# bioscan-ml/bioscan-clip

Hardware: AMD Instinct MI355X
Metric: paired samples/sec/node (I+D+T, global batch) + step MFMA-roofline % at 1/2/4/8 GPU (higher is better)
Workload: dtype bf16; 1 GPU; configs[2]: Image+DNA+Text (LoRA ViT-B/16 + LoRA BarcodeBERT + BERT-small), local batch 256, 224x224 images + 133-token barcodes, local-batch InfoNCE, fused AdamW; local_batch=256, global_batch=256, parallelism=dp1, collectives=none (one process, local-batch loss)

## Files before the change

### bioscan-clip_amd/csrc/optim.hip

```cpp
#include <math.h>

#include <type_traits>

#include "common.h"

namespace {

typedef __attribute__((ext_vector_type(4))) unsigned u32x4;

__device__ __forceinline__ f32x4 ld_bf4(const bf16_t* p) {
    const uint2 u = *reinterpret_cast<const uint2*>(p);
    return f32x4{bf2f(u.x & 0xffff), bf2f(u.x >> 16), bf2f(u.y & 0xffff), bf2f(u.y >> 16)};
}

__device__ __forceinline__ float reduce8(float (&p)[8], int lane) {
    float q[4];
    const bool hi5 = lane & 32;
#pragma unroll
    for (int i = 0; i < 4; ++i) {
        const float send = hi5 ? p[i] : p[i + 4];
        const float keep = hi5 ? p[i + 4] : p[i];
        q[i] = keep + __shfl_xor(send, 32, 64);
    }
    float r2[2];
    const bool hi4 = lane & 16;
#pragma unroll
    for (int i = 0; i < 2; ++i) {
        const float send = hi4 ? q[i] : q[i + 2];
        const float keep = hi4 ? q[i + 2] : q[i];
        r2[i] = keep + __shfl_xor(send, 16, 64);
    }
    const bool hi3 = lane & 8;
    float v = (hi3 ? r2[1] : r2[0]) + __shfl_xor(hi3 ? r2[0] : r2[1], 8, 64);
    v += __shfl_xor(v, 4, 64);
    v += __shfl_xor(v, 2, 64);
    v += __shfl_xor(v, 1, 64);
    return v;
}

constexpr int LG_BLOCK = 256;

__device__ __forceinline__ f32x4 splat4(float v) {
    f32x4 s = {v, v, v, v};
    asm("" : "+v"(s));
    return s;
}

__device__ __forceinline__ float reduce4(float (&p)[4], int lane) {
    float q[2];
    const bool hi5 = lane & 32;
#pragma unroll
    for (int i = 0; i < 2; ++i) {
        const float send = hi5 ? p[i] : p[i + 2];
        const float keep = hi5 ? p[i + 2] : p[i];
        q[i] = keep + __shfl_xor(send, 32, 64);
    }
    const bool hi4 = lane & 16;
    float v = (hi4 ? q[1] : q[0]) + __shfl_xor(hi4 ? q[0] : q[1], 16, 64);
    v += __shfl_xor(v, 8, 64);
    v += __shfl_xor(v, 4, 64);
    v += __shfl_xor(v, 2, 64);
    v += __shfl_xor(v, 1, 64);
    return v;
}

template <int H, bool F32IN = false>
__global__ __launch_bounds__(LG_BLOCK) void lora_grad_dt_db_kernel(const void* __restrict__ dqkv_, int ld,
                                                                    const void* __restrict__ haug_, int ld_h, int M,
                                                                    const float* __restrict__ lora_b,
                                                                    float* __restrict__ dt,
                                                                    float* __restrict__ partial) {
    const bf16_t* dqkv = static_cast<const bf16_t*>(dqkv_);
    const bf16_t* haug = static_cast<const bf16_t*>(haug_);
    constexpr int NV = H / 256;
    __shared__ float red[2 * NV * 16 * 64];
    const int lane = threadIdx.x & 63;
    const int wib = __builtin_amdgcn_readfirstlane(threadIdx.x >> 6);
    const int is_v = wib & 1;
    const int pair = blockIdx.x * (LG_BLOCK / 128) + (wib >> 1);
    const int npairs = gridDim.x * (LG_BLOCK / 128);
    for (int i = threadIdx.x; i < 2 * NV * 16 * 64; i += LG_BLOCK) red[i] = 0.f;

    f32x4 bx[NV][4];
    f32x4 ax[NV][4];
#pragma unroll
    for (int j = 0; j < NV; ++j)
#pragma unroll
        for (int i = 0; i < 4; ++i) {
            const int c = j * 256 + lane * 4 + i;
            bx[j][i] = *reinterpret_cast<const f32x4*>(lora_b + (size_t)(is_v * H + c) * 4);
            ax[j][i] = f32x4{0.f, 0.f, 0.f, 0.f};
        }

    constexpr int PF = 3;
    using row_t = std::conditional_t<F32IN, f32x4, uint2>;
    row_t rx[PF][NV];
    row_t rt[PF];
    auto fetch = [&](int slot, int row) {
        if constexpr (F32IN) {
            const float* g = static_cast<const float*>(dqkv_) + (size_t)row * ld + is_v * 2 * H;
#pragma unroll
            for (int j = 0; j < NV; ++j) rx[slot][j] = *reinterpret_cast<const f32x4*>(g + j * 256 + lane * 4);
            rt[slot] = *reinterpret_cast<const f32x4*>(static_cast<const float*>(haug_) + (size_t)row * ld_h + 4 * is_v);
        } else {
            const bf16_t* g = dqkv + (size_t)row * ld + is_v * 2 * H;
#pragma unroll
            for (int j = 0; j < NV; ++j) rx[slot][j] = *reinterpret_cast<const uint2*>(g + j * 256 + lane * 4);
            rt[slot] = *reinterpret_cast<const uint2*>(haug + (size_t)row * ld_h + H + 4 * is_v);
        }
    };
#pragma unroll
    for (int p = 0; p < PF; ++p)
        if (pair + p * npairs < M) fetch(p, pair + p * npairs);
    auto body = [&](int slot, int row) {
        f32x4 dx[NV];
        f32x4 tx;
        if constexpr (F32IN) {
#pragma unroll
            for (int j = 0; j < NV; ++j) dx[j] = rx[slot][j];
            tx = rt[slot];
        } else {
#pragma unroll
            for (int j = 0; j < NV; ++j)
                dx[j] = f32x4{bf2f(rx[slot][j].x & 0xffff), bf2f(rx[slot][j].x >> 16), bf2f(rx[slot][j].y & 0xffff),
                              bf2f(rx[slot][j].y >> 16)};
            const uint2 tu = rt[slot];
            tx = f32x4{bf2f(tu.x & 0xffff), bf2f(tu.x >> 16), bf2f(tu.y & 0xffff), bf2f(tu.y >> 16)};
        }
        if (row + PF * npairs < M) fetch(slot, row + PF * npairs);
        f32x4 px = {0.f, 0.f, 0.f, 0.f};
#pragma unroll
        for (int j = 0; j < NV; ++j)
#pragma unroll
            for (int i = 0; i < 4; ++i) {
                const f32x4 d4 = splat4(dx[j][i]);
                px += d4 * bx[j][i];
                ax[j][i] += d4 * tx;
            }
        float p[4] = {px[0], px[1], px[2], px[3]};
        const float tot = reduce4(p, lane);
        const float tl = __shfl(tot, ((lane >> 1) & 1) * 32 + (lane & 1) * 16, 64);
        if (lane < 4) dt[(size_t)row * 8 + 4 * is_v + lane] = tl;
    };
    for (int row = pair; row < M; row += PF * npairs) {
#pragma unroll
        for (int p = 0; p < PF; ++p)
            if (row + p * npairs < M) body(p, row + p * npairs);
    }
    float* mine = red + is_v * (NV * 16 * 64);
    for (int w = 0; w < LG_BLOCK / 64; ++w) {
        __syncthreads();
        if (wib == w) {
#pragma unroll
            for (int j = 0; j < NV; ++j)
#pragma unroll
                for (int i = 0; i < 4; ++i)
#pragma unroll
                    for (int r = 0; r < 4; ++r) mine[((j * 16 + i * 4 + r) * 64) + lane] += ax[j][i][r];
        }
    }
    __syncthreads();
    for (int idx = threadIdx.x; idx < 2 * NV * 16 * 64; idx += LG_BLOCK)
        partial[(size_t)blockIdx.x * (2 * NV * 16 * 64) + idx] = red[idx];
}

template <int H, bool Y_FP8 = false, bool Y_F32 = false, bool F16 = false>
__global__ __launch_bounds__(LG_BLOCK) void lora_grad_da_kernel(const void* __restrict__ haug_, int ld_h, int M,
                                                                 const float* __restrict__ dt,
                                                                 float* __restrict__ partial) {
    const bf16_t* haug = static_cast<const bf16_t*>(haug_);
    constexpr int NV = H / 256;
    __shared__ float red[8 * NV * 4 * 64];
    const int lane = threadIdx.x & 63;
    const int wave = (blockIdx.x * LG_BLOCK + threadIdx.x) >> 6;
    const int nwaves = (gridDim.x * LG_BLOCK) >> 6;
    for (int i = threadIdx.x; i < 8 * NV * 4 * 64; i += LG_BLOCK) red[i] = 0.f;
    f32x4 acc[8][NV];
#pragma unroll
    for (int r = 0; r < 8; ++r)
#pragma unroll
        for (int j = 0; j < NV; ++j) acc[r][j] = f32x4{0.f, 0.f, 0.f, 0.f};
    constexpr int PF = 3;
    for (int row0 = wave; row0 < M; row0 += PF * nwaves) {
        f32x4 d0[PF], d1[PF];
        std::conditional_t<Y_F32, f32x4, uint2> yr[PF][NV];
#pragma unroll
        for (int p = 0; p < PF; ++p) {
            const int row = min(row0 + p * nwaves, M - 1);
            d0[p] = *reinterpret_cast<const f32x4*>(dt + (size_t)row * 8);
            d1[p] = *reinterpret_cast<const f32x4*>(dt + (size_t)row * 8 + 4);
#pragma unroll
            for (int j = 0; j < NV; ++j) {
                if constexpr (Y_F32) {
                    yr[p][j] = *reinterpret_cast<const f32x4*>(static_cast<const float*>(haug_) + (size_t)row * ld_h + j * 256 + lane * 4);
                } else if constexpr (Y_FP8) {
                    yr[p][j].x = *reinterpret_cast<const unsigned*>(reinterpret_cast<const unsigned char*>(haug) +
                                                                    (size_t)row * ld_h + j * 256 + lane * 4);
                    yr[p][j].y = 0;
                } else {
                    yr[p][j] = *reinterpret_cast<const uint2*>(haug + (size_t)row * ld_h + j * 256 + lane * 4);
                }
            }
        }
#pragma unroll
        for (int p = 0; p < PF; ++p) {
            if (row0 + p * nwaves >= M) break;
#pragma unroll
            for (int j = 0; j < NV; ++j) {
                f32x4 y;
                if constexpr (Y_F32)
                    y = yr[p][j];
                else if constexpr (Y_FP8)
                    y = f32x4{fp8_to_f32(yr[p][j].x, 0), fp8_to_f32(yr[p][j].x, 1), fp8_to_f32(yr[p][j].x, 2), fp8_to_f32(yr[p][j].x, 3)};
                else
                    y = f32x4{h2f<F16>(yr[p][j].x & 0xffff), h2f<F16>(yr[p][j].x >> 16), h2f<F16>(yr[p][j].y & 0xffff),
                              h2f<F16>(yr[p][j].y >> 16)};
#pragma unroll
                for (int r = 0; r < 4; ++r) {
                    acc[r][j] += splat4(d0[p][r]) * y;
                    acc[4 + r][j] += splat4(d1[p][r]) * y;
                }
            }
        }
    }
    const int wib = threadIdx.x >> 6;
    for (int w = 0; w < LG_BLOCK / 64; ++w) {
        __syncthreads();
        if (wib == w) {
#pragma unroll
            for (int r = 0; r < 8; ++r)
#pragma unroll
                for (int j = 0; j < NV; ++j)
#pragma unroll
                    for (int i = 0; i < 4; ++i) red[(((r * NV + j) * 4 + i) * 64) + lane] += acc[r][j][i];
        }
    }
    __syncthreads();
    for (int idx = threadIdx.x; idx < 8 * NV * 4 * 64; idx += LG_BLOCK)
        partial[(size_t)blockIdx.x * (8 * NV * 4 * 64) + idx] = red[idx];
}

template <int H>
__global__ __launch_bounds__(LG_BLOCK) void lora_t_f32_kernel(const float* __restrict__ y, int ld_y, int M, const float* __restrict__ A,
                                                              float* __restrict__ t) {
    constexpr int NV = H / 256;
    __shared__ __attribute__((aligned(16))) float sA[8 * H];
    for (int i = threadIdx.x * 4; i < 8 * H; i += LG_BLOCK * 4) *reinterpret_cast<f32x4*>(sA + i) = *reinterpret_cast<const f32x4*>(A + i);
    __syncthreads();
    const int lane = threadIdx.x & 63;
    const int wave = (blockIdx.x * LG_BLOCK + threadIdx.x) >> 6, nwaves = (gridDim.x * LG_BLOCK) >> 6;
    for (int row = wave; row < M; row += nwaves) {
        asm volatile("" ::: "memory");
        f32x4 v[NV];
#pragma unroll
        for (int j = 0; j < NV; ++j) v[j] = *reinterpret_cast<const f32x4*>(y + (size_t)row * ld_y + j * 256 + lane * 4);
        float p[8];
#pragma unroll
        for (int r = 0; r < 8; ++r) {
            float d = 0.f;
#pragma unroll
            for (int j = 0; j < NV; ++j) {
                const f32x4 a = *reinterpret_cast<const f32x4*>(sA + r * H + j * 256 + lane * 4);
                d += (v[j][0] * a[0] + v[j][1] * a[1]) + (v[j][2] * a[2] + v[j][3] * a[3]);
            }
            p[r] = d;
        }
        const float tt = reduce8(p, lane);
        const float tl = __shfl(tt, ((lane >> 2) & 1) * 32 + ((lane >> 1) & 1) * 16 + (lane & 1) * 8, 64);
        if (lane < 8) t[(size_t)row * 8 + lane] = tl;
    }
}

template <int H, bool UNSCALE = false>
__global__ __launch_bounds__(256) void lora_grad_reduce_kernel(const float* __restrict__ pa,
                                                                const float* __restrict__ pb, int nblocks,
                                                                float* __restrict__ dA, float* __restrict__ dBq,
                                                                float* __restrict__ dBv, int first_block = 0, float unscale = 1.f) {
    constexpr int NV = H / 256;
    constexpr int SLAB = 8 * H;
    __shared__ f32x4 red[32][8];
    const int q = threadIdx.x & 7, p = threadIdx.x >> 3;
    const int idx = (blockIdx.x + first_block) * 32 + q * 4;
    const bool second = idx >= SLAB;
    const int e = second ? idx - SLAB : idx;
    const float* src = (second ? pb : pa) + e;
    f32x4 s = {0.f, 0.f, 0.f, 0.f};
    int b = p;
    for (; b + 96 < nblocks; b += 128) {
        f32x4 v[4];
#pragma unroll
        for (int u = 0; u < 4; ++u) v[u] = *reinterpret_cast<const f32x4*>(src + (size_t)(b + 32 * u) * SLAB);
#pragma unroll
        for (int u = 0; u < 4; ++u) s += v[u];
    }
    for (; b < nblocks; b += 32) s += *reinterpret_cast<const f32x4*>(src + (size_t)b * SLAB);
    red[p][q] = s;
    __syncthreads();
    if (p != 0) return;
    s = red[0][q];
#pragma unroll
    for (int g = 1; g < 32; ++g) s += red[g][q];
    if constexpr (UNSCALE) s *= unscale;
#pragma unroll
    for (int c = 0; c < 4; ++c) {
        const int ec = e + c;
        const int l = ec & 63, k = ec >> 6;
        if (!second) {
            const bool is_v = k >= NV * 16;
            const int kk = is_v ? k - NV * 16 : k;
            const int j = kk >> 4, ii = (kk >> 2) & 3, r = kk & 3;
            const int col = j * 256 + l * 4 + ii;
            float* dst = (is_v ? dBv : dBq) + (size_t)col * 4 + r;
            *dst += s[c];
        } else {
            const int ii = k & 3, j = (k >> 2) % NV, r = (k >> 2) / NV;
            dA[(size_t)r * H + j * 256 + l * 4 + ii] += s[c];
        }
    }
}

template <bool UNSCALE = false>
__global__ __launch_bounds__(256) void lora_heads_reduce_kernel(const float* __restrict__ dtp, const float* __restrict__ dbp, int M,
                                                                 int heads, int items, int nA, float* __restrict__ dt,
                                                                 float* __restrict__ dBq, float* __restrict__ dBv, float unscale = 1.f) {
    if ((int)blockIdx.x < nA) {
        const int g = blockIdx.x * 256 + threadIdx.x, row = g >> 1, half = g & 1;
        if (row >= M) return;
        f32x4 s = {0.f, 0.f, 0.f, 0.f};
        for (int hd = 0; hd < heads; hd += 4) {
            f32x4 v[4];
#pragma unroll
            for (int u = 0; u < 4; ++u) v[u] = *reinterpret_cast<const f32x4*>(dtp + (((size_t)(hd + u) * 2 + half) * M + row) * 4);
#pragma unroll
            for (int u = 0; u < 4; ++u) s += v[u];
        }
        *reinterpret_cast<f32x4*>(dt + (size_t)row * 8 + 4 * half) = s;
        return;
    }
    __shared__ float red[8][32];
    const int i = threadIdx.x & 31, p = threadIdx.x >> 5;
    const int e = ((int)blockIdx.x - nA) * 32 + i;
    const size_t stride = (size_t)heads * 512;
    const float* src = dbp + e;
    float s = 0.f;
    int b = p;
    for (; b + 56 < items; b += 64) {
        float v[8];
#pragma unroll
        for (int u = 0; u < 8; ++u) v[u] = src[(size_t)(b + 8 * u) * stride];
#pragma unroll
        for (int u = 0; u < 8; ++u) s += v[u];
    }
    for (; b < items; b += 8) s += src[(size_t)b * stride];
    red[p][i] = s;
    __syncthreads();
    if (p != 0) return;
    s = ((red[0][i] + red[1][i]) + (red[2][i] + red[3][i])) + ((red[4][i] + red[5][i]) + (red[6][i] + red[7][i]));
    if constexpr (UNSCALE) s *= unscale;
    const int hd = e >> 9, is_v = (e >> 8) & 1, j = (e >> 6) & 3, d = e & 63;
    float* dst = (is_v ? dBv : dBq) + (size_t)(hd * 64 + d) * 4 + j;
    *dst += s;
}

template <bool BF16>
__global__ __launch_bounds__(256) void colsum8_kernel(const void* __restrict__ g, int ld, int M, int N,
                                                       float* __restrict__ out) {
    __shared__ float part[256][9];
    __shared__ float part2[8][8];
    const int t = threadIdx.x;
    const int n0 = blockIdx.x * 8;
    float s[8] = {0.f, 0.f, 0.f, 0.f, 0.f, 0.f, 0.f, 0.f};
    auto add_row = [&](int r) {
        if constexpr (BF16) {
            const u32x4 u = *reinterpret_cast<const u32x4*>(static_cast<const bf16_t*>(g) + (size_t)r * ld + n0);
#pragma unroll
            for (int k = 0; k < 4; ++k) {
                s[2 * k] += bf2f(u[k] & 0xffff);
                s[2 * k + 1] += bf2f(u[k] >> 16);
            }
        } else {
            const float* p = static_cast<const float*>(g) + (size_t)r * ld + n0;
            const f32x4 a = *reinterpret_cast<const f32x4*>(p), b = *reinterpret_cast<const f32x4*>(p + 4);
#pragma unroll
            for (int k = 0; k < 4; ++k) {
                s[k] += a[k];
                s[4 + k] += b[k];
            }
        }
    };
    int r = t;
    for (; r + 768 < M; r += 1024) {
        add_row(r);
        add_row(r + 256);
        add_row(r + 512);
        add_row(r + 768);
    }
    for (; r < M; r += 256) add_row(r);
#pragma unroll
    for (int k = 0; k < 8; ++k) part[t][k] = s[k];
    __syncthreads();
    if (t < 64) {
        const int c = t & 7, o = t >> 3;
        float a = 0.f;
        for (int i = 0; i < 32; ++i) a += part[32 * o + i][c];
        part2[o][c] = a;
    }
    __syncthreads();
    if (t < 8) {
        float a = 0.f;
#pragma unroll
        for (int o = 0; o < 8; ++o) a += part2[o][t];
        out[n0 + t] += a;
    }
}

template <bool BF16>
__global__ __launch_bounds__(256) void colsum_kernel(const void* __restrict__ g, int ld, int M, int N,
                                                      float* __restrict__ out) {
    __shared__ float part[8][32];
    const int c = threadIdx.x & 31, rg = threadIdx.x >> 5;
    const int n = blockIdx.x * 32 + c;
    float s[4] = {0.f, 0.f, 0.f, 0.f};
    if (n < N) {
        auto at = [&](int r) -> float {
            if constexpr (BF16) return bf2f(static_cast<const bf16_t*>(g)[(size_t)r * ld + n]);
            else return static_cast<const float*>(g)[(size_t)r * ld + n];
        };
        int r = rg;
        for (; r + 24 < M; r += 32) {
#pragma unroll
            for (int u = 0; u < 4; ++u) s[u] += at(r + 8 * u);
        }
        for (; r < M; r += 8) s[0] += at(r);
    }
    part[rg][c] = (s[0] + s[1]) + (s[2] + s[3]);
    __syncthreads();
    if (rg == 0 && n < N) {
        float t = 0.f;
#pragma unroll
        for (int k = 0; k < 8; ++k) t += part[k][c];
        out[n] += t;
    }
}

__global__ __launch_bounds__(256) void adamw_kernel(float* __restrict__ p, const float* __restrict__ g,
                                                     float* __restrict__ m, float* __restrict__ v, long n, float lr,
                                                     float beta1, float beta2, float eps, float wd, float inv_bc1,
                                                     float inv_sqrt_bc2, float grad_scale) {
    for (long i = (long)blockIdx.x * 256 + threadIdx.x; i < n; i += (long)gridDim.x * 256) {
        const float gi = g[i] * grad_scale;
        float pi = p[i] * (1.0f - lr * wd);
        const float mi = beta1 * m[i] + (1.0f - beta1) * gi;
        const float vi = beta2 * v[i] + (1.0f - beta2) * gi * gi;
        const float denom = sqrtf(vi) * inv_sqrt_bc2 + eps;
        pi -= (lr * inv_bc1) * (mi / denom);
        p[i] = pi;
        m[i] = mi;
        v[i] = vi;
    }
}

__global__ __launch_bounds__(256) void adamw_dev_kernel(float* __restrict__ p, const float* __restrict__ g,
                                                         float* __restrict__ m, float* __restrict__ v, long n,
                                                         const float* __restrict__ hyper, float beta1, float beta2, float eps,
                                                         float wd, float grad_scale) {
    const float lr = hyper[0];
    const double step = (double)reinterpret_cast<const unsigned*>(hyper)[1];
    const float inv_bc1 = (float)(1.0 / (1.0 - pow((double)beta1, step)));
    const float inv_sqrt_bc2 = (float)(1.0 / sqrt(1.0 - pow((double)beta2, step)));
    for (long i = (long)blockIdx.x * 256 + threadIdx.x; i < n; i += (long)gridDim.x * 256) {
        const float gi = g[i] * grad_scale;
        float pi = p[i] * (1.0f - lr * wd);
        const float mi = beta1 * m[i] + (1.0f - beta1) * gi;
        const float vi = beta2 * v[i] + (1.0f - beta2) * gi * gi;
        const float denom = sqrtf(vi) * inv_sqrt_bc2 + eps;
        pi -= (lr * inv_bc1) * (mi / denom);
        p[i] = pi;
        m[i] = mi;
        v[i] = vi;
    }
}

}

constexpr int LG_MAX_BLOCKS = 768;

extern "C" int64_t bsclip_lora_grad_workspace_floats(int H) { return (int64_t)LG_MAX_BLOCKS * 16 * H; }

extern "C" int bsclip_lora_grad(const void* dqkv, int ld_dqkv, const void* h, int ld_h, int M, int H,
                                const float* lora_b, float* dt, float* dA, float* dBq, float* dBv, float* workspace,
                                void* stream) {
    BSCLIP_REQUIRE(dqkv && h && lora_b && dt && dA && dBq && dBv && workspace && M > 0,
                   "bsclip_lora_grad: null/empty input");
    BSCLIP_REQUIRE(H == 768 || H == 512, "bsclip_lora_grad: H=%d (supported: 768, 512)", H);
    BSCLIP_REQUIRE(ld_dqkv >= 3 * H && ld_dqkv % 4 == 0 && ld_h >= H + 8 && ld_h % 8 == 0,
                   "bsclip_lora_grad: ld_dqkv=%d ld_h=%d", ld_dqkv, ld_h);
    hipStream_t s = static_cast<hipStream_t>(stream);
    int blocks = ceil_div(M, 4 * 8);
    if (blocks > LG_MAX_BLOCKS) blocks = LG_MAX_BLOCKS;
    if (blocks < 1) blocks = 1;
    const bf16_t* g = static_cast<const bf16_t*>(dqkv);
    const bf16_t* hh = static_cast<const bf16_t*>(h);
    float* pa = workspace;
    float* pb = workspace + (size_t)LG_MAX_BLOCKS * 8 * H;
    if (H == 768) {
        hipLaunchKernelGGL((lora_grad_dt_db_kernel<768>), dim3(blocks), dim3(LG_BLOCK), 0, s, g, ld_dqkv, hh, ld_h, M,
                           lora_b, dt, pa);
        hipLaunchKernelGGL((lora_grad_da_kernel<768>), dim3(blocks), dim3(LG_BLOCK), 0, s, hh, ld_h, M, dt, pb);
        hipLaunchKernelGGL((lora_grad_reduce_kernel<768>), dim3(16 * 768 / 32), dim3(256), 0, s, pa, pb,
                           blocks, dA, dBq, dBv);
    } else {
        hipLaunchKernelGGL((lora_grad_dt_db_kernel<512>), dim3(blocks), dim3(LG_BLOCK), 0, s, g, ld_dqkv, hh, ld_h, M,
                           lora_b, dt, pa);
        hipLaunchKernelGGL((lora_grad_da_kernel<512>), dim3(blocks), dim3(LG_BLOCK), 0, s, hh, ld_h, M, dt, pb);
        hipLaunchKernelGGL((lora_grad_reduce_kernel<512>), dim3(16 * 512 / 32), dim3(256), 0, s, pa, pb,
                           blocks, dA, dBq, dBv);
    }
    BSCLIP_LAUNCH_CHECK();
    return BSCLIP_OK;
}

extern "C" int bsclip_lora_grad_heads(const void* h, int ld_h, int M, int H, int B, const float* dt_partial,
                                      const float* db_partial, float* dt, float* dA, float* dBq, float* dBv, float* workspace,
                                      void* stream) {
    BSCLIP_REQUIRE(h && dt_partial && db_partial && dt && dA && dBq && dBv && workspace && M > 0 && B > 0 && M % B == 0,
                   "bsclip_lora_grad_heads: null/empty input (M=%d B=%d)", M, B);
    BSCLIP_REQUIRE(H == 768 || H == 512, "bsclip_lora_grad_heads: H=%d (supported: 768, 512)", H);
    BSCLIP_REQUIRE(ld_h >= H && ld_h % 8 == 0, "bsclip_lora_grad_heads: ld_h=%d", ld_h);
    BSCLIP_REQUIRE(((reinterpret_cast<uintptr_t>(dt_partial) | reinterpret_cast<uintptr_t>(dt)) & 15) == 0,
                   "bsclip_lora_grad_heads: dt_partial and dt must be 16-byte aligned");
    hipStream_t s = static_cast<hipStream_t>(stream);
    const int heads = H / 64;
    int blocks = ceil_div(M, 4 * 8);
    if (blocks > LG_MAX_BLOCKS) blocks = LG_MAX_BLOCKS;
    if (blocks < 1) blocks = 1;
    const bf16_t* hh = static_cast<const bf16_t*>(h);
    float* pb = workspace + (size_t)LG_MAX_BLOCKS * 8 * H;
    const int nA = ceil_div(2 * M, 256);
    hipLaunchKernelGGL(lora_heads_reduce_kernel<false>, dim3(nA + heads * 512 / 32), dim3(256), 0, s, dt_partial, db_partial, M, heads, B, nA,
                       dt, dBq, dBv);
    if (H == 768) {
        hipLaunchKernelGGL((lora_grad_da_kernel<768>), dim3(blocks), dim3(LG_BLOCK), 0, s, hh, ld_h, M, dt, pb);
        hipLaunchKernelGGL((lora_grad_reduce_kernel<768>), dim3(8 * 768 / 32), dim3(256), 0, s, (const float*)nullptr, pb, blocks, dA,
                           dBq, dBv, 8 * 768 / 32);
    } else {
        hipLaunchKernelGGL((lora_grad_da_kernel<512>), dim3(blocks), dim3(LG_BLOCK), 0, s, hh, ld_h, M, dt, pb);
        hipLaunchKernelGGL((lora_grad_reduce_kernel<512>), dim3(8 * 512 / 32), dim3(256), 0, s, (const float*)nullptr, pb, blocks, dA,
                           dBq, dBv, 8 * 512 / 32);
    }
    BSCLIP_LAUNCH_CHECK();
    return BSCLIP_OK;
}

extern "C" int bsclip_lora_grad_heads_f16(const void* h, int ld_h, int M, int H, int B, const float* dt_partial,
                                          const float* db_partial, float* dt, float* dA, float* dBq, float* dBv, float* workspace,
                                          int operands, void* stream) {
    bool f16 = false;
    BSCLIP_REQUIRE(take_operands_flag(operands, f16), "bsclip_lora_grad_heads_f16: unknown bits in operands=0x%x", operands);
    BSCLIP_REQUIRE(f16 && operands <= 64, "bsclip_lora_grad_heads_f16: operands=0x%x must be BSCLIP_OPERANDS_FP16 | s, s <= 64",
                   operands);
    BSCLIP_REQUIRE(h && dt_partial && db_partial && dt && dA && dBq && dBv && workspace && M > 0 && B > 0 && M % B == 0,
                   "bsclip_lora_grad_heads_f16: null/empty input (M=%d B=%d)", M, B);
    BSCLIP_REQUIRE(H == 768, "bsclip_lora_grad_heads_f16: H=%d (the ViT's 768)", H);
    BSCLIP_REQUIRE(ld_h >= H && ld_h % 8 == 0, "bsclip_lora_grad_heads_f16: ld_h=%d", ld_h);
    BSCLIP_REQUIRE(((reinterpret_cast<uintptr_t>(dt_partial) | reinterpret_cast<uintptr_t>(dt) | reinterpret_cast<uintptr_t>(workspace) |
                     reinterpret_cast<uintptr_t>(h)) & 15) == 0,
                   "bsclip_lora_grad_heads_f16: h, dt_partial, dt and workspace must be 16-byte aligned");
    hipStream_t s = static_cast<hipStream_t>(stream);
    const float unscale = ldexpf(1.f, -operands);
    const int heads = H / 64;
    int blocks = ceil_div(M, 4 * 8);
    if (blocks > LG_MAX_BLOCKS) blocks = LG_MAX_BLOCKS;
    if (blocks < 1) blocks = 1;
    const bf16_t* hh = static_cast<const bf16_t*>(h);
    float* pb = workspace + (size_t)LG_MAX_BLOCKS * 8 * H;
    const int nA = ceil_div(2 * M, 256);
    hipLaunchKernelGGL(lora_heads_reduce_kernel<true>, dim3(nA + heads * 512 / 32), dim3(256), 0, s, dt_partial, db_partial, M, heads, B,
                       nA, dt, dBq, dBv, unscale);
    hipLaunchKernelGGL((lora_grad_da_kernel<768, false, false, true>), dim3(blocks), dim3(LG_BLOCK), 0, s, hh, ld_h, M, dt, pb);
    hipLaunchKernelGGL((lora_grad_reduce_kernel<768, true>), dim3(8 * 768 / 32), dim3(256), 0, s, (const float*)nullptr, pb, blocks, dA,
                       dBq, dBv, 8 * 768 / 32, unscale);
    BSCLIP_LAUNCH_CHECK();
    return BSCLIP_OK;
}

__global__ __launch_bounds__(256) void add_scaled_f32_kernel(const float* __restrict__ in, long n, float scale, float* __restrict__ out) {
    const long n4 = n >> 2;
    for (long i = (long)blockIdx.x * 256 + threadIdx.x; i < n4; i += (long)gridDim.x * 256) {
        const f32x4 v = *reinterpret_cast<const f32x4*>(in + 4 * i);
        f32x4 o = *reinterpret_cast<const f32x4*>(out + 4 * i);
        o += v * scale;
        *reinterpret_cast<f32x4*>(out + 4 * i) = o;
    }
    if (blockIdx.x == 0 && threadIdx.x < (n & 3)) {
        const long i = (n4 << 2) + threadIdx.x;
        out[i] += in[i] * scale;
    }
}

extern "C" int bsclip_add_scaled_f32(const float* in, int64_t n, int scale_log2, float* out, void* stream) {
    BSCLIP_REQUIRE(in && out && n > 0, "bsclip_add_scaled_f32: bad args");
    BSCLIP_REQUIRE(scale_log2 >= -64 && scale_log2 <= 64, "bsclip_add_scaled_f32: scale_log2=%d (|k| <= 64)", scale_log2);
    BSCLIP_REQUIRE(((reinterpret_cast<uintptr_t>(in) | reinterpret_cast<uintptr_t>(out)) & 15) == 0,
                   "bsclip_add_scaled_f32: in and out must be 16-byte aligned");
    long blocks = (n / 4 + 255) / 256;
    if (blocks < 1) blocks = 1;
    if (blocks > 1024) blocks = 1024;
    hipLaunchKernelGGL(add_scaled_f32_kernel, dim3((unsigned)blocks), dim3(256), 0, static_cast<hipStream_t>(stream), in, (long)n,
                       ldexpf(1.f, scale_log2), out);
    BSCLIP_LAUNCH_CHECK();
    return BSCLIP_OK;
}

extern "C" int64_t bsclip_lora_grad_f32_workspace_floats(int M, int H) {
    return M > 0 && H > 0 ? 16 * (int64_t)((M + 3) / 4 * 4) + (int64_t)LG_MAX_BLOCKS * 16 * H : -1;
}

extern "C" int bsclip_lora_grad_f32(const float* dqkv, int ld_dqkv, const float* y, int ld_y, int M, int H, const float* lora_a,
                                    const float* lora_b, float* dA, float* dB, float* workspace, void* stream) {
    BSCLIP_REQUIRE(dqkv && y && lora_a && lora_b && dA && dB && workspace, "bsclip_lora_grad_f32: null pointer");
    BSCLIP_REQUIRE(M > 0 && (H == 768 || H == 512) && ld_dqkv >= 3 * H && ld_dqkv % 4 == 0 && ld_y >= H && ld_y % 4 == 0,
                   "bsclip_lora_grad_f32: M=%d H=%d ld_dqkv=%d ld_y=%d", M, H, ld_dqkv, ld_y);
    BSCLIP_REQUIRE(((reinterpret_cast<uintptr_t>(dqkv) | reinterpret_cast<uintptr_t>(y) | reinterpret_cast<uintptr_t>(lora_a) |
                     reinterpret_cast<uintptr_t>(lora_b) | reinterpret_cast<uintptr_t>(workspace)) & 15) == 0,
                   "bsclip_lora_grad_f32: dqkv, y, lora_a, lora_b and workspace must be 16-byte aligned (vector loads)");
    hipStream_t s = static_cast<hipStream_t>(stream);
    int blocks = ceil_div(M, 4 * 8);
    if (blocks > LG_MAX_BLOCKS) blocks = LG_MAX_BLOCKS;
    if (blocks < 1) blocks = 1;
    const size_t Mp = (size_t)(M + 3) / 4 * 4;
    float* t = workspace;
    float* dt = workspace + 8 * Mp;
    float* pa = workspace + 16 * Mp;
    float* pb = pa + (size_t)LG_MAX_BLOCKS * 8 * H;
    float* dBq = dB;
    float* dBv = dB + (size_t)H * 4;
    if (H == 768) {
        hipLaunchKernelGGL((lora_t_f32_kernel<768>), dim3(blocks), dim3(LG_BLOCK), 0, s, y, ld_y, M, lora_a, t);
        hipLaunchKernelGGL((lora_grad_dt_db_kernel<768, true>), dim3(blocks), dim3(LG_BLOCK), 0, s, dqkv, ld_dqkv, t, 8, M, lora_b, dt, pa);
        hipLaunchKernelGGL((lora_grad_da_kernel<768, false, true>), dim3(blocks), dim3(LG_BLOCK), 0, s, y, ld_y, M, dt, pb);
        hipLaunchKernelGGL((lora_grad_reduce_kernel<768>), dim3(16 * 768 / 32), dim3(256), 0, s, pa, pb, blocks, dA, dBq, dBv);
    } else {
        hipLaunchKernelGGL((lora_t_f32_kernel<512>), dim3(blocks), dim3(LG_BLOCK), 0, s, y, ld_y, M, lora_a, t);
        hipLaunchKernelGGL((lora_grad_dt_db_kernel<512, true>), dim3(blocks), dim3(LG_BLOCK), 0, s, dqkv, ld_dqkv, t, 8, M, lora_b, dt, pa);
        hipLaunchKernelGGL((lora_grad_da_kernel<512, false, true>), dim3(blocks), dim3(LG_BLOCK), 0, s, y, ld_y, M, dt, pb);
        hipLaunchKernelGGL((lora_grad_reduce_kernel<512>), dim3(16 * 512 / 32), dim3(256), 0, s, pa, pb, blocks, dA, dBq, dBv);
    }
    BSCLIP_LAUNCH_CHECK();
    return BSCLIP_OK;
}

extern "C" int bsclip_lora_grad_fp8(const void* dqkv, int ld_dqkv, const void* y_fp8, int ld_y, const void* t_aug, int ld_t,
                                    int M, int H, const float* lora_b, float* dt, float* dA, float* dBq, float* dBv,
                                    float* workspace, void* stream) {
    BSCLIP_REQUIRE(dqkv && y_fp8 && t_aug && lora_b && dt && dA && dBq && dBv && workspace && M > 0,
                   "bsclip_lora_grad_fp8: null/empty input");
    BSCLIP_REQUIRE(H == 768 || H == 512, "bsclip_lora_grad_fp8: H=%d (supported: 768, 512)", H);
    BSCLIP_REQUIRE(ld_dqkv >= 3 * H && ld_dqkv % 4 == 0 && ld_y >= H && ld_y % 4 == 0 && ld_t >= 8 && ld_t % 8 == 0,
                   "bsclip_lora_grad_fp8: ld_dqkv=%d ld_y=%d ld_t=%d", ld_dqkv, ld_y, ld_t);
    hipStream_t s = static_cast<hipStream_t>(stream);
    int blocks = ceil_div(M, 4 * 8);
    if (blocks > LG_MAX_BLOCKS) blocks = LG_MAX_BLOCKS;
    if (blocks < 1) blocks = 1;
    const bf16_t* g = static_cast<const bf16_t*>(dqkv);
    const bf16_t* tt = static_cast<const bf16_t*>(t_aug) - H;
    const bf16_t* yy = static_cast<const bf16_t*>(y_fp8);
    float* pa = workspace;
    float* pb = workspace + (size_t)LG_MAX_BLOCKS * 8 * H;
    if (H == 768) {
        hipLaunchKernelGGL((lora_grad_dt_db_kernel<768>), dim3(blocks), dim3(LG_BLOCK), 0, s, g, ld_dqkv, tt, ld_t, M, lora_b, dt, pa);
        hipLaunchKernelGGL((lora_grad_da_kernel<768, true>), dim3(blocks), dim3(LG_BLOCK), 0, s, yy, ld_y, M, dt, pb);
        hipLaunchKernelGGL((lora_grad_reduce_kernel<768>), dim3(16 * 768 / 32), dim3(256), 0, s, pa, pb, blocks, dA, dBq, dBv);
    } else {
        hipLaunchKernelGGL((lora_grad_dt_db_kernel<512>), dim3(blocks), dim3(LG_BLOCK), 0, s, g, ld_dqkv, tt, ld_t, M, lora_b, dt, pa);
        hipLaunchKernelGGL((lora_grad_da_kernel<512, true>), dim3(blocks), dim3(LG_BLOCK), 0, s, yy, ld_y, M, dt, pb);
        hipLaunchKernelGGL((lora_grad_reduce_kernel<512>), dim3(16 * 512 / 32), dim3(256), 0, s, pa, pb, blocks, dA, dBq, dBv);
    }
    BSCLIP_LAUNCH_CHECK();
    return BSCLIP_OK;
}

extern "C" int bsclip_colsum(const void* g, int ld_g, int g_is_bf16, int M, int N, float* out, void* stream) {
    BSCLIP_REQUIRE(g && out && M > 0 && N > 0 && ld_g >= N, "bsclip_colsum: bad args");
    hipStream_t s = static_cast<hipStream_t>(stream);
    const bool wide = N % 8 == 0 && ld_g % 8 == 0 && (((uintptr_t)g) & 15) == 0;
    if (wide) {
        if (g_is_bf16) hipLaunchKernelGGL((colsum8_kernel<true>), dim3(N / 8), dim3(256), 0, s, g, ld_g, M, N, out);
        else hipLaunchKernelGGL((colsum8_kernel<false>), dim3(N / 8), dim3(256), 0, s, g, ld_g, M, N, out);
    } else {
        const dim3 grid(ceil_div(N, 32));
        if (g_is_bf16) hipLaunchKernelGGL((colsum_kernel<true>), grid, dim3(256), 0, s, g, ld_g, M, N, out);
        else hipLaunchKernelGGL((colsum_kernel<false>), grid, dim3(256), 0, s, g, ld_g, M, N, out);
    }
    BSCLIP_LAUNCH_CHECK();
    return BSCLIP_OK;
}

extern "C" int bsclip_adamw_step(float* p, const float* g, float* m, float* v, int64_t n, float lr, float beta1,
                                 float beta2, float eps, float weight_decay, int step, float grad_scale,
                                 void* stream) {
    BSCLIP_REQUIRE(p && g && m && v && n > 0 && step >= 1, "bsclip_adamw_step: bad args (n=%ld step=%d)", (long)n, step);
    const double bc1 = 1.0 - pow((double)beta1, (double)step);
    const double bc2 = 1.0 - pow((double)beta2, (double)step);
    long blocks = (n + 255) / 256;
    if (blocks > 2048) blocks = 2048;
    hipLaunchKernelGGL(adamw_kernel, dim3((unsigned)blocks), dim3(256), 0, static_cast<hipStream_t>(stream), p, g, m, v,
                       (long)n, lr, beta1, beta2, eps, weight_decay, (float)(1.0 / bc1), (float)(1.0 / sqrt(bc2)),
                       grad_scale);
    BSCLIP_LAUNCH_CHECK();
    return BSCLIP_OK;
}

extern "C" int bsclip_adamw_step_dev(float* p, const float* g, float* m, float* v, int64_t n, const float* hyper_dev,
                                     float beta1, float beta2, float eps, float weight_decay, float grad_scale, void* stream) {
    BSCLIP_REQUIRE(p && g && m && v && hyper_dev && n > 0, "bsclip_adamw_step_dev: null/empty input");
    long blocks = (n + 255) / 256;
    if (blocks > 2048) blocks = 2048;
    hipLaunchKernelGGL(adamw_dev_kernel, dim3((unsigned)blocks), dim3(256), 0, static_cast<hipStream_t>(stream), p, g, m, v,
                       (long)n, hyper_dev, beta1, beta2, eps, weight_decay, grad_scale);
    BSCLIP_LAUNCH_CHECK();
    return BSCLIP_OK;
}
```

Measured before the change: 6560 paired samples/s.

## Fuse LoRA head-sum of dt into dA kernel and merge tail reductions

Adds a heads variant of the LoRA dA-gradient kernel. Each block first sums the per-head dt partials for the rows it will process, writes dt, and stages those values in shared memory. The block then runs the dA outer-product loop with the next rows' activations prefetched, instead of reading dt back from global memory. The dB reduction and the dA slab reduction are merged into one tail kernel, so the LoRA backward tail goes from three launches to two. The fused path is taken only when the rows per wave fit the shared staging chunk, and it can be disabled with an environment variable.

Measured after the change: 6576 paired samples/s (median of 6 runs). About the same (+0.2%).

```diff
diff --git a/bioscan-clip_amd/csrc/optim.hip b/bioscan-clip_amd/csrc/optim.hip
--- a/bioscan-clip_amd/csrc/optim.hip
+++ b/bioscan-clip_amd/csrc/optim.hip
@@ -164,13 +164,17 @@
         partial[(size_t)blockIdx.x * (2 * NV * 16 * 64) + idx] = red[idx];
 }
 
-template <int H, bool Y_FP8 = false, bool Y_F32 = false, bool F16 = false>
-__global__ __launch_bounds__(LG_BLOCK) void lora_grad_da_kernel(const void* __restrict__ haug_, int ld_h, int M,
-                                                                 const float* __restrict__ dt,
-                                                                 float* __restrict__ partial) {
+constexpr int DA_PF = 3;
+constexpr int DA_CHUNK = 30;
+template <int H, bool Y_FP8, bool Y_F32, bool F16, bool HEADS>
+__device__ __forceinline__ void lora_grad_da_body(const void* __restrict__ haug_, int ld_h, int M, const float* __restrict__ dt,
+                                                  float* __restrict__ partial, float* __restrict__ dt_out) {
+    static_assert(!HEADS || (H / 64) % 4 == 0, "the head sum takes four heads at a time");
+    static_assert(DA_CHUNK % DA_PF == 0 && DA_CHUNK * 8 <= LG_BLOCK && LG_BLOCK == 256, "head-sum round: one thread per (iteration, wave, half)");
     const bf16_t* haug = static_cast<const bf16_t*>(haug_);
     constexpr int NV = H / 256;
     __shared__ float red[8 * NV * 4 * 64];
+    __shared__ __attribute__((aligned(16))) float sdt[HEADS ? DA_CHUNK * 4 * 8 : 4];
     const int lane = threadIdx.x & 63;
     const int wave = (blockIdx.x * LG_BLOCK + threadIdx.x) >> 6;
     const int nwaves = (gridDim.x * LG_BLOCK) >> 6;
@@ -180,15 +184,20 @@
     for (int r = 0; r < 8; ++r)
 #pragma unroll
         for (int j = 0; j < NV; ++j) acc[r][j] = f32x4{0.f, 0.f, 0.f, 0.f};
-    constexpr int PF = 3;
-    for (int row0 = wave; row0 < M; row0 += PF * nwaves) {
-        f32x4 d0[PF], d1[PF];
-        std::conditional_t<Y_F32, f32x4, uint2> yr[PF][NV];
+    constexpr int PF = DA_PF;
+    using yrow_t = std::conditional_t<Y_F32, f32x4, uint2>;
+    auto load_dt = [&](int row0, f32x4 (&d0)[PF], f32x4 (&d1)[PF]) {
 #pragma unroll
         for (int p = 0; p < PF; ++p) {
             const int row = min(row0 + p * nwaves, M - 1);
             d0[p] = *reinterpret_cast<const f32x4*>(dt + (size_t)row * 8);
             d1[p] = *reinterpret_cast<const f32x4*>(dt + (size_t)row * 8 + 4);
+        }
+    };
+    auto load_y = [&](int row0, yrow_t (&yr)[PF][NV]) {
+#pragma unroll
+        for (int p = 0; p < PF; ++p) {
+            const int row = min(row0 + p * nwaves, M - 1);
 #pragma unroll
             for (int j = 0; j < NV; ++j) {
                 if constexpr (Y_F32) {
@@ -202,6 +211,8 @@
                 }
             }
         }
+    };
+    auto products = [&](int row0, const yrow_t (&yr)[PF][NV], const f32x4 (&d0)[PF], const f32x4 (&d1)[PF]) {
 #pragma unroll
         for (int p = 0; p < PF; ++p) {
             if (row0 + p * nwaves >= M) break;
@@ -222,8 +233,49 @@
                 }
             }
         }
-    }
+    };
     const int wib = threadIdx.x >> 6;
+    if constexpr (HEADS) {
+        constexpr int HEADS_N = H / 64;
+        const int wave0 = blockIdx.x * (LG_BLOCK / 64);
+        const int kr = threadIdx.x >> 3, sw = (threadIdx.x >> 1) & 3, half = threadIdx.x & 1;
+        yrow_t yr[PF][NV];
+        load_y(wave, yr);
+        const long srow = (long)wave0 + sw + (long)kr * nwaves;
+        if (kr < DA_CHUNK && srow < M) {
+            f32x4 s = {0.f, 0.f, 0.f, 0.f};
+#pragma unroll
+            for (int hd = 0; hd < HEADS_N; hd += 4) {
+                f32x4 v[4];
+#pragma unroll
+                for (int u = 0; u < 4; ++u) v[u] = *reinterpret_cast<const f32x4*>(dt + (((size_t)(hd + u) * 2 + half) * M + srow) * 4);
+#pragma unroll
+                for (int u = 0; u < 4; ++u) s += v[u];
+            }
+            *reinterpret_cast<f32x4*>(dt_out + (size_t)srow * 8 + 4 * half) = s;
+            *reinterpret_cast<f32x4*>(sdt + ((kr * 4 + sw) * 2 + half) * 4) = s;
+        }
+        __syncthreads();
+        const float* dsrc = sdt + wib * 8;
+        for (int row0 = wave; row0 < M; row0 += PF * nwaves, dsrc += PF * 4 * 8) {
+            f32x4 d0[PF], d1[PF];
+#pragma unroll
+            for (int p = 0; p < PF; ++p) {
+                d0[p] = *reinterpret_cast<const f32x4*>(dsrc + p * 4 * 8);
+                d1[p] = *reinterpret_cast<const f32x4*>(dsrc + p * 4 * 8 + 4);
+            }
+            products(row0, yr, d0, d1);
+            if (row0 + PF * nwaves < M) load_y(row0 + PF * nwaves, yr);
+        }
+    } else {
+        for (int row0 = wave; row0 < M; row0 += PF * nwaves) {
+            f32x4 d0[PF], d1[PF];
+            yrow_t yr[PF][NV];
+            load_dt(row0, d0, d1);
+            load_y(row0, yr);
+            products(row0, yr, d0, d1);
+        }
+    }
     for (int w = 0; w < LG_BLOCK / 64; ++w) {
         __syncthreads();
         if (wib == w) {
@@ -238,6 +290,20 @@
     __syncthreads();
     for (int idx = threadIdx.x; idx < 8 * NV * 4 * 64; idx += LG_BLOCK)
         partial[(size_t)blockIdx.x * (8 * NV * 4 * 64) + idx] = red[idx];
+}
+
+template <int H, bool Y_FP8 = false, bool Y_F32 = false, bool F16 = false>
+__global__ __launch_bounds__(LG_BLOCK) void lora_grad_da_kernel(const void* __restrict__ haug_, int ld_h, int M,
+                                                                 const float* __restrict__ dt,
+                                                                 float* __restrict__ partial) {
+    lora_grad_da_body<H, Y_FP8, Y_F32, F16, false>(haug_, ld_h, M, dt, partial, nullptr);
+}
+
+template <int H, bool F16 = false>
+__global__ __launch_bounds__(LG_BLOCK) void lora_grad_da_heads_kernel(const void* __restrict__ haug_, int ld_h, int M,
+                                                                       const float* __restrict__ dt_partial,
+                                                                       float* __restrict__ partial, float* __restrict__ dt) {
+    lora_grad_da_body<H, false, false, F16, true>(haug_, ld_h, M, dt_partial, partial, dt);
 }
 
 template <int H>
@@ -271,16 +337,15 @@
     }
 }
 
-template <int H, bool UNSCALE = false>
-__global__ __launch_bounds__(256) void lora_grad_reduce_kernel(const float* __restrict__ pa,
-                                                                const float* __restrict__ pb, int nblocks,
-                                                                float* __restrict__ dA, float* __restrict__ dBq,
-                                                                float* __restrict__ dBv, int first_block = 0, float unscale = 1.f) {
+template <int H, bool UNSCALE>
+__device__ __forceinline__ void lora_slab_reduce_block(int blk, const float* __restrict__ pa, const float* __restrict__ pb, int nblocks,
+                                                       float* __restrict__ dA, float* __restrict__ dBq, float* __restrict__ dBv,
+                                                       float unscale) {
     constexpr int NV = H / 256;
     constexpr int SLAB = 8 * H;
     __shared__ f32x4 red[32][8];
     const int q = threadIdx.x & 7, p = threadIdx.x >> 3;
-    const int idx = (blockIdx.x + first_block) * 32 + q * 4;
+    const int idx = blk * 32 + q * 4;
     const bool second = idx >= SLAB;
     const int e = second ? idx - SLAB : idx;
     const float* src = (second ? pb : pa) + e;
@@ -319,6 +384,42 @@
     }
 }
 
+template <int H, bool UNSCALE = false>
+__global__ __launch_bounds__(256) void lora_grad_reduce_kernel(const float* __restrict__ pa,
+                                                                const float* __restrict__ pb, int nblocks,
+                                                                float* __restrict__ dA, float* __restrict__ dBq,
+                                                                float* __restrict__ dBv, int first_block = 0, float unscale = 1.f) {
+    lora_slab_reduce_block<H, UNSCALE>((int)blockIdx.x + first_block, pa, pb, nblocks, dA, dBq, dBv, unscale);
+}
+
+template <bool UNSCALE>
+__device__ __forceinline__ void lora_heads_db_block(int blk, const float* __restrict__ dbp, int heads, int items, float* __restrict__ dBq,
+                                                    float* __restrict__ dBv, float unscale) {
+    __shared__ float red[8][32];
+    const int i = threadIdx.x & 31, p = threadIdx.x >> 5;
+    const int e = blk * 32 + i;
+    const size_t stride = (size_t)heads * 512;
+    const float* src = dbp + e;
+    float s = 0.f;
+    int b = p;
+    for (; b + 56 < items; b += 64) {
+        float v[8];
+#pragma unroll
+        for (int u = 0; u < 8; ++u) v[u] = src[(size_t)(b + 8 * u) * stride];
+#pragma unroll
+        for (int u = 0; u < 8; ++u) s += v[u];
+    }
+    for (; b < items; b += 8) s += src[(size_t)b * stride];
+    red[p][i] = s;
+    __syncthreads();
+    if (p != 0) return;
+    s = ((red[0][i] + red[1][i]) + (red[2][i] + red[3][i])) + ((red[4][i] + red[5][i]) + (red[6][i] + red[7][i]));
+    if constexpr (UNSCALE) s *= unscale;
+    const int hd = e >> 9, is_v = (e >> 8) & 1, j = (e >> 6) & 3, d = e & 63;
+    float* dst = (is_v ? dBv : dBq) + (size_t)(hd * 64 + d) * 4 + j;
+    *dst += s;
+}
+
 template <bool UNSCALE = false>
 __global__ __launch_bounds__(256) void lora_heads_reduce_kernel(const float* __restrict__ dtp, const float* __restrict__ dbp, int M,
                                                                  int heads, int items, int nA, float* __restrict__ dt,
@@ -337,29 +438,15 @@
         *reinterpret_cast<f32x4*>(dt + (size_t)row * 8 + 4 * half) = s;
         return;
     }
-    __shared__ float red[8][32];
-    const int i = threadIdx.x & 31, p = threadIdx.x >> 5;
-    const int e = ((int)blockIdx.x - nA) * 32 + i;
-    const size_t stride = (size_t)heads * 512;
-    const float* src = dbp + e;
-    float s = 0.f;
-    int b = p;
-    for (; b + 56 < items; b += 64) {
-        float v[8];
-#pragma unroll
-        for (int u = 0; u < 8; ++u) v[u] = src[(size_t)(b + 8 * u) * stride];
-#pragma unroll
-        for (int u = 0; u < 8; ++u) s += v[u];
-    }
-    for (; b < items; b += 8) s += src[(size_t)b * stride];
-    red[p][i] = s;
-    __syncthreads();
-    if (p != 0) return;
-    s = ((red[0][i] + red[1][i]) + (red[2][i] + red[3][i])) + ((red[4][i] + red[5][i]) + (red[6][i] + red[7][i]));
-    if constexpr (UNSCALE) s *= unscale;
-    const int hd = e >> 9, is_v = (e >> 8) & 1, j = (e >> 6) & 3, d = e & 63;
-    float* dst = (is_v ? dBv : dBq) + (size_t)(hd * 64 + d) * 4 + j;
-    *dst += s;
+    lora_heads_db_block<UNSCALE>((int)blockIdx.x - nA, dbp, heads, items, dBq, dBv, unscale);
+}
+
+template <int H, bool UNSCALE = false>
+__global__ __launch_bounds__(256) void lora_tail_reduce_kernel(const float* __restrict__ dbp, int heads, int items, int nDB,
+                                                                const float* __restrict__ pb, int nblocks, float* __restrict__ dA,
+                                                                float* __restrict__ dBq, float* __restrict__ dBv, float unscale = 1.f) {
+    if ((int)blockIdx.x < nDB) lora_heads_db_block<UNSCALE>((int)blockIdx.x, dbp, heads, items, dBq, dBv, unscale);
+    else lora_slab_reduce_block<H, UNSCALE>((int)blockIdx.x - nDB + 8 * H / 32, nullptr, pb, nblocks, dA, dBq, dBv, unscale);
 }
 
 template <bool BF16>
@@ -520,6 +607,11 @@
     return BSCLIP_OK;
 }
 
+static bool lora_tail_fused(int M, int blocks) {
+    const char* v = getenv("BSCLIP_LORA_TAIL_FUSED");
+    return !(v && atoi(v) == 0) && ceil_div(M, blocks * (LG_BLOCK / 64)) <= DA_CHUNK;
+}
+
 extern "C" int bsclip_lora_grad_heads(const void* h, int ld_h, int M, int H, int B, const float* dt_partial,
                                       const float* db_partial, float* dt, float* dA, float* dBq, float* dBv, float* workspace,
                                       void* stream) {
@@ -527,8 +619,8 @@
                    "bsclip_lora_grad_heads: null/empty input (M=%d B=%d)", M, B);
     BSCLIP_REQUIRE(H == 768 || H == 512, "bsclip_lora_grad_heads: H=%d (supported: 768, 512)", H);
     BSCLIP_REQUIRE(ld_h >= H && ld_h % 8 == 0, "bsclip_lora_grad_heads: ld_h=%d", ld_h);
-    BSCLIP_REQUIRE(((reinterpret_cast<uintptr_t>(dt_partial) | reinterpret_cast<uintptr_t>(dt)) & 15) == 0,
-                   "bsclip_lora_grad_heads: dt_partial and dt must be 16-byte aligned");
+    BSCLIP_REQUIRE(((reinterpret_cast<uintptr_t>(dt_partial) | reinterpret_cast<uintptr_t>(dt) | reinterpret_cast<uintptr_t>(workspace)) & 15) == 0,
+                   "bsclip_lora_grad_heads: dt_partial, dt and workspace must be 16-byte aligned");
     hipStream_t s = static_cast<hipStream_t>(stream);
     const int heads = H / 64;
     int blocks = ceil_div(M, 4 * 8);
@@ -537,6 +629,22 @@
     const bf16_t* hh = static_cast<const bf16_t*>(h);
     float* pb = workspace + (size_t)LG_MAX_BLOCKS * 8 * H;
     const int nA = ceil_div(2 * M, 256);
+    if (lora_tail_fused(M, blocks)) {
+        const int nDB = heads * 512 / 32;
+        if (H == 768) {
+            hipLaunchKernelGGL((lora_grad_da_heads_kernel<768>), dim3(blocks), dim3(LG_BLOCK), 0, s, hh, ld_h, M,
+                               dt_partial, pb, dt);
+            hipLaunchKernelGGL((lora_tail_reduce_kernel<768>), dim3(nDB + 8 * 768 / 32), dim3(256), 0, s, db_partial, heads, B, nDB, pb,
+                               blocks, dA, dBq, dBv);
+        } else {
+            hipLaunchKernelGGL((lora_grad_da_heads_kernel<512>), dim3(blocks), dim3(LG_BLOCK), 0, s, hh, ld_h, M,
+                               dt_partial, pb, dt);
+            hipLaunchKernelGGL((lora_tail_reduce_kernel<512>), dim3(nDB + 8 * 512 / 32), dim3(256), 0, s, db_partial, heads, B, nDB, pb,
+                               blocks, dA, dBq, dBv);
+        }
+        BSCLIP_LAUNCH_CHECK();
+        return BSCLIP_OK;
+    }
     hipLaunchKernelGGL(lora_heads_reduce_kernel<false>, dim3(nA + heads * 512 / 32), dim3(256), 0, s, dt_partial, db_partial, M, heads, B, nA,
                        dt, dBq, dBv);
     if (H == 768) {
@@ -575,6 +683,15 @@
     const bf16_t* hh = static_cast<const bf16_t*>(h);
     float* pb = workspace + (size_t)LG_MAX_BLOCKS * 8 * H;
     const int nA = ceil_div(2 * M, 256);
+    if (lora_tail_fused(M, blocks)) {
+        const int nDB = heads * 512 / 32;
+        hipLaunchKernelGGL((lora_grad_da_heads_kernel<768, true>), dim3(blocks), dim3(LG_BLOCK), 0, s, hh, ld_h, M, dt_partial,
+                           pb, dt);
+        hipLaunchKernelGGL((lora_tail_reduce_kernel<768, true>), dim3(nDB + 8 * 768 / 32), dim3(256), 0, s, db_partial, heads, B, nDB, pb,
+                           blocks, dA, dBq, dBv, unscale);
+        BSCLIP_LAUNCH_CHECK();
+        return BSCLIP_OK;
+    }
     hipLaunchKernelGGL(lora_heads_reduce_kernel<true>, dim3(nA + heads * 512 / 32), dim3(256), 0, s, dt_partial, db_partial, M, heads, B,
                        nA, dt, dBq, dBv, unscale);
     hipLaunchKernelGGL((lora_grad_da_kernel<768, false, false, true>), dim3(blocks), dim3(LG_BLOCK), 0, s, hh, ld_h, M, dt, pb);
```
